# juliuspleunes4/TurboInfer

Hardware: AMD Instinct MI355X
Metric: decode tokens/s/GPU, Llama-7B-shape INT4 @2048 ctx; % HBM-read roofline (higher is better)
Workload: dtype w4a16; 1 GPU; llama2-7b INT4 g128 decode, 1 stream(s)/GPU, KV 2048, replay at pos 2047; model=llama2-7b, global_batch=1, seq_len=2048, parallelism=replicas1 (request-sharded, no collectives)

## Files before the change

include/ti_hip.h:

```cpp
#ifndef TI_HIP_H
#define TI_HIP_H

#include <stddef.h>
#include <stdint.h>

#ifdef __cplusplus
extern "C" {
#endif

typedef void* ti_stream_t;

enum ti_status {
  TI_OK = 0,
  TI_ERR_ARG = 1,
  TI_ERR_HIP = 2,
  TI_ERR_UNSUPPORTED = 3,
  TI_ERR_NOMEM = 4,
  TI_ERR_NODEV = 5
};

const char* ti_last_error(void);

int ti_device_count(int* count);
int ti_init(int device);
// ... 125 lines not shown
                      int max_seq, const int32_t* pos, int M, int heads, int kv_heads, int head_dim, int splits,
                      float* workspace, uint16_t* out, ti_stream_t s);
int ti_attn_decode_packed_f8(const float* q, const uint8_t* k_cache, const uint8_t* v_cache,
                             int64_t kv_stream_stride, int max_seq, const int32_t* pos, int M, int heads,
                             int kv_heads, int head_dim, int splits, float* workspace, uint16_t* out,
                             ti_stream_t s);
int ti_attn_decode_partials_f8(const float* q, const uint8_t* k_cache, const uint8_t* v_cache,
                               int64_t kv_stream_stride, int max_seq, const int32_t* pos, int M, int heads,
                               int kv_heads, int head_dim, int splits, uint16_t* part_o, float* part_ml,
                               ti_stream_t s);
int ti_qkv_attn_partials(const void* tiles, const uint16_t* scales, int bits, const uint16_t* fx,
                         const float* ss_in, int n_ss, float eps, const float* rope_cs, const int32_t* pos,
                         uint16_t* k_cache, uint16_t* v_cache, int max_seq, int K, int heads, int kv_heads,
                         int head_dim, int splits, uint16_t* part_o, float* part_ml, void* xchg, ti_stream_t s);
size_t ti_qkv_attn_part_o_elems(int heads, int head_dim, int splits);
size_t ti_qkv_attn_part_ml_elems(int heads, int head_dim, int splits);
size_t ti_qkv_attn_xchg_bytes(int heads, int splits);
size_t ti_qkv_attn_error_offset(int heads, int splits);
int ti_qkv_attn_supported(int bits, int K, int heads, int kv_heads, int head_dim, int splits);
int ti_attn_prefill(const float* q, const uint16_t* k_cache, const uint16_t* v_cache, int max_seq,
                    const int32_t* pos, int M, int heads, int kv_heads, int head_dim, uint16_t* out,
                    ti_stream_t s);
int ti_attn_prefill_f8(const float* q, const uint8_t* k_cache, const uint8_t* v_cache, int max_seq,
                       const int32_t* pos, int M, int heads, int kv_heads, int head_dim, uint16_t* out,
                       ti_stream_t s);
size_t ti_attn_prefill_split_workspace_bytes(int M, int heads, int head_dim, int splits);
int ti_attn_prefill_split(const float* q, const uint16_t* k_cache, const uint16_t* v_cache, int max_seq,
                          const int32_t* pos, int M, int heads, int kv_heads, int head_dim, int splits,
                          float* workspace, uint16_t* out, ti_stream_t s);
int ti_attn_prefill_set_kernel(int mode);

int ti_gemm_kernel_name(int bits, int x_kind, int M, int N, int K, char* buf, int len);

int ti_hbm_calibrate(size_t bytes, int reps, double* read_gbps, double* copy_gbps, ti_stream_t s);


typedef struct ti_step_args {
  const uint16_t* emb;
  float* h;
  int32_t hidden, M, vocab, in_stride, out_stride, placeholder_first;
  const int32_t* in_tokens;
  const int32_t* n_in;
  unsigned long long* argmax;
  int32_t* out_tokens;
  int32_t* pos;
  const int32_t* base_pos;
  const int32_t* step_ctr;
  const float* fold_w;
  uint16_t* fold_x;
  float* fold_ss;
} ti_step_args;
int ti_step_begin(const ti_step_args* a, ti_stream_t s);

#define TI_LA_STATE_WORDS 8
#define TI_LA_MAX_K 15
#define TI_LA_MAX_NGRAM 8
typedef struct ti_lookahead_args {
  int32_t* state;
  const int32_t* cfg;
  int32_t* hist;
  int32_t k, hidden, vocab, max_pos;
  const uint16_t* emb;
  float* h;
  int32_t* row_tok;
  int32_t* pos;
  unsigned long long* argmax;
// ... 41 lines not shown
```

turboinfer_amd/__init__.py:

```python
from __future__ import annotations

import ctypes as C
import os
import subprocess

import numpy as np

HERE = os.path.dirname(os.path.abspath(__file__))
ROOT = os.path.dirname(HERE)
LIB_PATH = os.environ.get("TI_LIB") or os.path.join(HERE, "lib", "libturboinfer_amd.so")

TI_OK = 0
X_F16, X_F32, X_F32_RMSNORM, X_F16_FOLDED, X_ATTN_SPLITS, X_F16_PACKED = 0, 1, 2, 3, 4, 5
ATTN_MAX_PART_SPLITS = 8
EPI_STORE_F32, EPI_STORE_F16, EPI_RESID_F32, EPI_SILU_MUL_F16, EPI_QKV_ROPE_KV, EPI_LOGITS_ARGMAX = range(6)
ARGMAX_SLOTS = 32
GEMM_MAX_ROWS = 1024
BITS_G32 = 32
BITS_AFF = 64
BITS_KV8 = 128
SCALE_GROUP, SCALE_TENSOR, SCALE_UNIT = 0, 1, 2
ROWS_CONCAT, ROWS_INTERLEAVE8 = 0, 1
(W_Q, W_K, W_V, W_O, W_GATE, W_UP, W_DOWN, W_LM_HEAD, V_ATTN_NORM, V_FFN_NORM, V_OUT_NORM, E_EMBED) = range(12)

# ... 39 lines not shown
                ("rope_theta", C.c_float), ("eps", C.c_float), ("bits", C.c_int32), ("max_seq", C.c_int32),
                ("max_batch", C.c_int32), ("compat", C.c_int32), ("device", C.c_int32),
                ("attn_splits", C.c_int32)]


EXPORTED = [
    "ti_last_error", "ti_device_count", "ti_init", "ti_device_name", "ti_malloc", "ti_free", "ti_memcpy_h2d",
    "ti_memcpy_d2h", "ti_memcpy_d2d", "ti_memset", "ti_stream_create", "ti_stream_destroy", "ti_stream_sync",
    "ti_device_sync", "ti_event_create", "ti_event_destroy", "ti_event_record", "ti_event_elapsed_ms",
    "ti_wpack_tile_bytes", "ti_wpack_scale_bytes", "ti_wpack_host", "ti_wsynth_device", "ti_fill_uniform_f16",
    "ti_fill_uniform_f32", "ti_fill_kv_uniform", "ti_kv_copy_slots", "ti_gemm_wq_a16", "ti_gemm_lds_bytes", "ti_gemm_prepare",
    "ti_gemm_max_rows", "ti_gemm_packed_rows", "ti_gemm_packed_rows_for", "ti_gemm_tile_plan", "ti_rmsnorm_f16", "ti_rmsnorm_f16_packed", "ti_attn_decode_packed", "ti_attn_prefill", "ti_attn_prefill_set_kernel",
    "ti_attn_workspace_bytes", "ti_attn_decode", "ti_step_begin", "ti_matmul_f32", "ti_rms_norm_f32",
    "ti_rope_f32", "ti_silu_f32", "ti_relu_f32", "ti_add_f32", "ti_mul_f32", "ti_softmax_f32", "ti_attention_f32",
    "ti_argmax_f32", "ti_engine_create", "ti_engine_destroy", "ti_engine_get_stream", "ti_engine_memory", "ti_engine_set_tensor",
    "ti_engine_synth", "ti_engine_fill_kv", "ti_engine_generate", "ti_engine_step", "ti_engine_compat_step",
    "ti_engine_replay_prepare", "ti_engine_set_prefill", "ti_engine_replay_run", "ti_engine_sync", "ti_engine_last_tokens",
    "ti_engine_time_kernel", "ti_engine_stamp_steps", "ti_rope_table", "ti_sample_token", 
    "ti_gemm_grid", "ti_engine_set_fold",
    "ti_attn_decode_partials", "ti_sample_device", "ti_sample_step", "ti_engine_generate_sampled",
    "ti_engine_beam_search", "ti_engine_serve", 
    "ti_wpack_q_host", "ti_engine_set_tensor_q", "ti_sample_workspace_bytes", "ti_sample_device_ws",
    "ti_wpack_q1_host", "ti_engine_set_tensor_q1", "ti_epilogue_bytes",
    "ti_sample_step_ws", "ti_hbm_calibrate", "ti_gemm_kernel_name",
    "ti_gemm_fold_partials", "ti_engine_set_stop", "ti_engine_counters",
    "ti_qkv_attn_partials", "ti_qkv_attn_part_o_elems", "ti_qkv_attn_part_ml_elems", "ti_engine_set_qkv_attn",
    "ti_qkv_attn_xchg_bytes", "ti_qkv_attn_supported", "ti_qkv_attn_error_offset",
    "ti_logprob_rows", "ti_engine_score",
    "ti_attn_decode_f8", "ti_attn_decode_packed_f8", "ti_attn_decode_partials_f8", "ti_fill_kv_uniform_f8",
    "ti_attn_prefill_f8", "ti_engine_prefill_attn_name",
    "ti_engine_read_kv",
    "ti_attn_prefill_split", "ti_attn_prefill_split_workspace_bytes", "ti_lookahead_begin", "ti_lookahead_accept",
    "ti_engine_generate_lookahead",
]

_lib = None


def build(jobs: int = 8) -> None:
    subprocess.run(["make", "-s", "-C", ROOT, f"-j{jobs}", "all"], check=True)


def lib() -> C.CDLL:
    global _lib
    if _lib is None:
        if not os.path.exists(LIB_PATH):
            raise TiError(f"native library missing: {LIB_PATH} (run `make` or __graft_entry__.build())")
        L = C.CDLL(LIB_PATH)
        vp, i32, i64, u64, f32, sz = C.c_void_p, C.c_int, C.c_int64, C.c_uint64, C.c_float, C.c_size_t
        L.ti_last_error.restype = C.c_char_p
        L.ti_device_count.argtypes = [C.POINTER(C.c_int)]
        L.ti_init.argtypes = [i32]
        L.ti_device_name.argtypes = [i32, C.c_char_p, i32]
        L.ti_malloc.argtypes = [C.POINTER(vp), sz]
        L.ti_free.argtypes = [vp]
        for n in ("ti_memcpy_h2d", "ti_memcpy_d2h", "ti_memcpy_d2d"):
            getattr(L, n).argtypes = [vp, vp, sz, vp]
        L.ti_memset.argtypes = [vp, i32, sz, vp]
        L.ti_stream_sync.argtypes = [vp]
        L.ti_wpack_tile_bytes.argtypes = [i32, i32, i32]
        L.ti_wpack_tile_bytes.restype = sz
        L.ti_wpack_scale_bytes.argtypes = [i32, i32, i32]
        L.ti_wpack_scale_bytes.restype = sz
        L.ti_wpack_host.argtypes = [vp, i32, i32, i32, i32, i32, i32, i32, vp, vp]
        L.ti_wsynth_device.argtypes = [u64, C.c_uint32, i32, i32, i32, i32, i32, i32, vp, vp, vp]
        L.ti_fill_uniform_f16.argtypes = [u64, C.c_uint32, u64, f32, vp, vp]
# ... 64 lines not shown
            L.ti_engine_set_fold.argtypes = [vp, i32, C.POINTER(C.c_int)]
        if hasattr(L, "ti_qkv_attn_partials"):
            L.ti_engine_set_qkv_attn.argtypes = [vp, i32, C.POINTER(C.c_int)]
            L.ti_qkv_attn_partials.argtypes = [vp, vp, i32, vp, vp, i32, f32, vp, vp, vp, vp, i32, i32, i32, i32,
                                               i32, i32, vp, vp, vp, vp]
            L.ti_qkv_attn_xchg_bytes.argtypes = [i32, i32]
            L.ti_qkv_attn_supported.argtypes = [i32, i32, i32, i32, i32, i32]
            L.ti_qkv_attn_xchg_bytes.restype = sz
            L.ti_qkv_attn_error_offset.argtypes = [i32, i32]
            L.ti_qkv_attn_error_offset.restype = sz
            L.ti_qkv_attn_part_o_elems.argtypes = [i32, i32, i32]
            L.ti_qkv_attn_part_o_elems.restype = sz
            L.ti_qkv_attn_part_ml_elems.argtypes = [i32, i32, i32]
            L.ti_qkv_attn_part_ml_elems.restype = sz
        if hasattr(L, "ti_engine_score"):
            L.ti_logprob_rows.argtypes = [vp, i32, i32, i32, vp, vp, vp, vp]
            L.ti_engine_score.argtypes = [vp, i32, vp, i32, i32, vp, vp, vp]
        if hasattr(L, "ti_attn_decode_f8"):
            for n in ("ti_attn_decode_f8", "ti_attn_decode_packed_f8", "ti_attn_decode_partials_f8"):
                getattr(L, n).argtypes = [vp, vp, vp, i64, i32, vp, i32, i32, i32, i32, i32, vp, vp, vp]
            L.ti_fill_kv_uniform_f8.argtypes = [u64, C.c_uint32, i32, i32, i32, i32, vp, vp]
            L.ti_engine_read_kv.argtypes = [vp, i32, i32, i32, i32, i32, vp]
        if hasattr(L, "ti_attn_prefill_f8"):
            L.ti_attn_prefill_f8.argtypes = [vp, vp, vp, i32, vp, i32, i32, i32, i32, vp, vp]
            L.ti_engine_prefill_attn_name.argtypes = [vp, i32, C.c_char_p, i32]
        if hasattr(L, "ti_engine_generate_lookahead"):
            L.ti_attn_prefill_split.argtypes = [vp, vp, vp, i32, vp, i32, i32, i32, i32, i32, vp, vp, vp]
            L.ti_attn_prefill_split_workspace_bytes.argtypes = [i32, i32, i32, i32]
            L.ti_attn_prefill_split_workspace_bytes.restype = sz
            L.ti_lookahead_begin.argtypes = [C.POINTER(LookaheadArgs), vp]
            L.ti_lookahead_accept.argtypes = [C.POINTER(LookaheadArgs), vp]
            L.ti_engine_generate_lookahead.argtypes = [vp, i32, vp, i32, i32, vp, i32, i32, i32, i32, vp,
                                                       C.POINTER(LookaheadStats)]
        L.ti_engine_compat_step.argtypes = [vp, i32, vp]
        L.ti_engine_replay_prepare.argtypes = [vp, i32, i32, i32]
        L.ti_engine_replay_run.argtypes = [vp, i32]
        L.ti_engine_sync.argtypes = [vp]
        L.ti_engine_last_tokens.argtypes = [vp, i32, vp]
        L.ti_engine_time_kernel.argtypes = [vp, i32, i32, i32, i32, C.POINTER(C.c_double), C.POINTER(C.c_double)]
        if hasattr(L, "ti_engine_stamp_steps"):
            L.ti_engine_stamp_steps.argtypes = [vp, i32, i32, vp, vp, C.POINTER(C.c_int)]
        L.ti_hbm_calibrate.argtypes = [sz, i32, C.POINTER(C.c_double), C.POINTER(C.c_double), vp]
        L.ti_gemm_kernel_name.argtypes = [i32, i32, i32, i32, i32, C.c_char_p, i32]
        L.ti_rope_table.argtypes = [vp, i32, i32, f32, vp]
        L.ti_sample_token.argtypes = [vp, i32, f32, i32, f32, f32, C.POINTER(C.c_int), C.POINTER(C.c_float)]
        _lib = L
    return _lib


def check(rc: int) -> None:
    if rc != TI_OK:
        raise TiError(f"ti error {rc}: {lib().ti_last_error().decode()}")


def device_count() -> int:
    n = C.c_int(0)
    check(lib().ti_device_count(C.byref(n)))
    return n.value


def init(device: int = 0) -> None:
    check(lib().ti_init(device))


def _ptr(a: np.ndarray) -> C.c_void_p:
    return C.c_void_p(a.ctypes.data)
# ... 311 lines not shown
```

turboinfer_amd/csrc/kernels/gemv.hip:

```cpp
#include <math.h>
#include <atomic>
#include <stdlib.h>

#include "common.hpp"
#include "attention_body.hpp"
#include "dequant.hpp"

namespace ti {

typedef uint32_t u32x4 __attribute__((ext_vector_type(4)));

#ifndef TI_GEMV_RING_VGPRS
#define TI_GEMV_RING_VGPRS 20
#endif
#ifndef TI_GEMV_SYNC
#define TI_GEMV_SYNC 0
#endif
#ifndef TI_GEMV_RING_DELAY
#define TI_GEMV_RING_DELAY 0
#endif
#ifndef TI_GEMV_EXP
#define TI_GEMV_EXP 0
#endif
#if TI_GEMV_EXP & 4
__device__ unsigned long long g_gemv_ts[4096 * 8];
#define GEMV_TS(k) \
  do { if (threadIdx.x == 0) g_gemv_ts[blockIdx.x * 8 + (k)] = __builtin_amdgcn_s_memrealtime(); } while (0)
__device__ unsigned long long g_gemv_wts[4096 * 8];
#define GEMV_WTS() \
  do { if ((threadIdx.x & 63) == 0) g_gemv_wts[blockIdx.x * 8 + (threadIdx.x >> 6)] = __builtin_amdgcn_s_memrealtime(); } while (0)
__device__ unsigned long long g_rows_ts[4096 * 8 * 8];
#define ROWS_TS(k)                                                                                     \
  do {                                                                                                 \
    if ((threadIdx.x & 63) == 0)                                                                       \
      g_rows_ts[(blockIdx.x * 8 + (threadIdx.x >> 6)) * 8 + (k)] = __builtin_amdgcn_s_memrealtime();   \
  } while (0)
#else
#define GEMV_WTS() do { } while (0)
#define GEMV_TS(k) do { } while (0)
#define ROWS_TS(k) do { } while (0)
#endif

constexpr int kGemvWaves = 8;
constexpr int kGemvThreads = kGemvWaves * kWave;

struct GemvArgs {
  const u32x4* tiles;
  const uint16_t* scales;
  const void* x;
  const float* norm_w;
  float eps;
  int32_t x_kind, ldx, M, N, K;
  ti_epilogue epi;
  unsigned long long* stamp;
};

__host__ __device__ constexpr int align16(int b) { return (b + 15) & ~15; }

struct GemmKnobs {
  bool splitk = true;
  bool rows_split = true;
};
__host__ inline const GemmKnobs& gemm_knobs() {
  static const GemmKnobs k = [] {
    GemmKnobs v;
    if (const char* e = getenv("TI_GEMM_SPLITK")) v.splitk = atoi(e) != 0;
    if (const char* e = getenv("TI_GEMM_ROWS_SPLIT")) v.rows_split = atoi(e) != 0;
    return v;
  }();
  return k;
}


__host__ __device__ inline int gemv_lds_bytes_tiles(int M, int K, int tiles_per_wg, bool g32 = false, bool aff = false);

__host__ inline int gemv_grid(int M, int N, int K, int num_cus, bool g32 = false, bool aff = false) {
  const int NT = N >> 4;
  const int g = num_cus > 0 ? num_cus : 256;
  int grid = NT < g ? NT : g;
  while (grid < NT && gemv_lds_bytes_tiles(M, K, (NT + grid - 1) / grid, g32, aff) > 160 * 1024) grid += grid / 8 + 1;
  return grid < NT ? grid : NT;
}

struct GemvLds {
  int x, sc, corr, slab, es, best, total, mins, bsum;
};
__host__ __device__ inline GemvLds gemv_lds_layout(int M, int K, int ntl, bool g32 = false, bool aff = false) {
  GemvLds l;
  const int gm = g32 ? 4 : 1;
  l.x = 0;
  l.sc = l.x + align16(M * (K + 8) * 2);
  l.mins = l.sc + align16(ntl * (K >> 7) * 32 * gm);
  l.corr = l.mins + (aff ? align16(ntl * (K >> 7) * 32 * gm) : 0);
  l.bsum = l.corr + (K >> 7) * 16 * 4 * gm;
  l.slab = l.bsum + (aff ? (K >> 7) * 16 * 4 * gm : 0);
  l.es = l.slab + (ntl + 1) * kGemvWaves * kWave * 16;
  const int es_bytes = 2 * ntl * M * 16 * 4 > M * 128 * 4 + 64 ? 2 * ntl * M * 16 * 4 : M * 128 * 4 + 64;
  l.best = l.es + align16(es_bytes);
  l.total = l.best + 16 * 8;
  return l;
// ... 124 lines not shown
      }
      break;
    }
    default:
      break;
  }
}

#ifndef TI_GEMV_NT
#define TI_GEMV_NT 1
#endif
__device__ __forceinline__ u32x4 ld_w(const u32x4* p) {
#if TI_GEMV_NT || (TI_GEMV_EXP & 16)
  return __builtin_nontemporal_load(p);
#else
  return *p;
#endif
}

__device__ __forceinline__ float int4_x_prep(f16x8& h) {
  const f16 s16 = (f16)0.0625f;
  h[2] *= s16; h[3] *= s16; h[6] *= s16; h[7] *= s16;
  const float lo = ((float)h[0] + (float)h[1]) + ((float)h[4] + (float)h[5]);
  const float hi = ((float)h[2] + (float)h[3]) + ((float)h[6] + (float)h[7]);
  return 1032.0f * lo + 1152.0f * hi;
}

__device__ __forceinline__ void lds_barrier() {
  asm volatile("s_waitcnt lgkmcnt(0)" ::: "memory");
  __builtin_amdgcn_s_barrier();
  asm volatile("" ::: "memory");
}

template <int BITS, int XM, bool G32 = false, bool AFF = false>
__global__ __launch_bounds__(kGemvThreads, 1) void gemv_wq_kernel(const u32x4* p_tiles, const uint16_t* p_scales,
                                                                   const void* p_x, const float* p_aux, int p_mgk,
                                                                   int p_N, int p_kx, int p_ldo, const float* p_pre,
                                                                   GemvArgs a) {
  const unsigned long long t_entry = stamp_now();
  const unsigned bid = blockIdx.x;
  a.tiles = p_tiles;
  a.scales = p_scales;
  a.x = p_x;
  a.norm_w = p_aux;
  a.M = p_mgk & 63;
  const int nt_q = p_N & 0xff, nt_r = (int)((unsigned)p_N >> 8);
  a.K = p_kx & 0xffff;
  a.ldx = XM == XM_F16F || XM == XM_ATTN ? a.K : (int)((unsigned)p_kx >> 16);
  const int p_grid = (p_mgk >> 6) & 0xfff;
  a.N = 16 * (nt_q * p_grid + nt_r);
  constexpr int C = TileFmt<BITS>::kChunks;
  constexpr int R = TI_GEMV_RING_VGPRS / (4 * C) > 2 ? TI_GEMV_RING_VGPRS / (4 * C) : 2;
  constexpr int XPF = 3;
  extern __shared__ __attribute__((aligned(16))) char smem[];
  GEMV_TS(0);
  const int KT = a.K >> 7, xs = a.K + 8, NT = a.N >> 4, K8 = a.K >> 3;
  const int tid = threadIdx.x, lane = tid & 63;
  const int wave = __builtin_amdgcn_readfirstlane(tid >> 6);
  const int t0 = (int)bid * nt_q + ((int)bid < nt_r ? (int)bid : nt_r);
  const int ntl = nt_q + ((int)bid < nt_r ? 1 : 0);
  constexpr bool kOneRow = XM == XM_F16F || XM == XM_ATTN || XM == XM_NORM1;
  const int KW = wave < KT ? (KT - wave + kGemvWaves - 1) / kGemvWaves : 0;
  const int total = ntl * KW;
  static_assert(!G32 || BITS != 16, "group-32 weights: int4 / int8");
  static_assert(!AFF || (G32 && BITS == 4), "affine blocks: group-32 int4");
  const GemvLds L = gemv_lds_layout(a.M, a.K, ntl, G32, AFF);
  uint16_t* ml = (uint16_t*)(smem + L.mins);
// ... 27 lines not shown
  u32x4 po[XM == XM_ATTN ? kPS : 1];
  float2 pml[XM == XM_ATTN ? kPS : 1];
  auto load_x = [&]() {
    if constexpr (XM == XM_ATTN) {
      const int S = (int)((unsigned)p_kx >> 16), hsh = ((p_mgk >> 21) & 3) == 2 ? 7 : 6;
      const int i = tid < K8 ? tid : K8 - 1, h = (8 * i) >> hsh, d = (8 * i) & ((1 << hsh) - 1);
#pragma unroll
      for (int sp = 0; sp < kPS; ++sp) {
        const int r = h * S + (sp < S ? sp : S - 1);
        po[sp] = *(const u32x4*)((const f16*)a.x + ((size_t)r << hsh) + d);
        pml[sp] = *(const float2*)(p_aux + 2 * r);
      }
    } else if constexpr (XM == XM_NORM1) {
      const int k8 = tid < K8 ? tid : K8 - 1;
      const float* xr = (const float*)a.x;
      v0 = *(const float4*)(xr + 8 * k8);
      v1 = *(const float4*)(xr + 8 * k8 + 4);
    } else if constexpr (XM == XM_F16 || XM == XM_F16F) {
#pragma unroll
      for (int q = 0; q < XPF; ++q) {
        const int i = tid + q * kGemvThreads < nx16 ? tid + q * kGemvThreads : nx16 - 1;
        const int m = kOneRow ? 0 : i / K8, k8 = i - m * K8;
        xr16[q] = *(const u32x4*)((const f16*)a.x + (size_t)m * a.ldx + 8 * k8);
      }
    }
  };
  if constexpr (XM == XM_NORM1) {
#endif
    const int k8 = tid < K8 ? tid : K8 - 1;
    w0 = *(const float4*)(a.norm_w + 8 * k8);
    w1 = *(const float4*)(a.norm_w + 8 * k8 + 4);
  }
  load_x();
  const int kind = (p_mgk >> 18) & 7, ldo = p_ldo;
  const int n_res = kind == TI_EPI_RESID_F32 ? ntl * a.M * 16 : 0;
  const float* pre_p;
  {
    const int idx = tid < n_res ? tid : 0;
    const int tl = kOneRow ? idx >> 4 : idx / (a.M * 16), rem = idx - tl * a.M * 16, m = rem >> 4, n = rem & 15;
    pre_p = kind == TI_EPI_RESID_F32 ? p_pre + (size_t)m * ldo + (t0 + tl) * 16 + n
            : kind == TI_EPI_QKV_ROPE_KV ? p_pre + (tid < a.M ? tid : 0) : p_pre;
  }
  const float pre = *pre_p;
  float fw_pre = 0.0f;
  float ss4[4] = {0.0f, 0.0f, 0.0f, 0.0f};
  const int n_ss = (int)((unsigned)p_kx >> 16);
  if constexpr (XM == XM_F16F) {
#pragma unroll
    for (int j = 0; j < 4; ++j) ss4[j] = p_aux[lane + 64 * j < n_ss ? lane + 64 * j : 0];
  }

  const u32x4* tb = a.tiles + (size_t)t0 * KT * (kWave * C) + lane;
  const size_t last_off = total > 0 ? ((size_t)(ntl - 1) * KT + wave + kGemvWaves * (KW - 1)) * (kWave * C) : 0;
  int rt = 0, rk = 0, rj = 0;
  auto refill_off = [&]() -> size_t {
    const size_t o = rj < total ? ((size_t)rt * KT + wave + kGemvWaves * rk) * (kWave * C) : last_off;
    ++rj;
    if (++rk == KW) { rk = 0; ++rt; }
    return o;
  };
  constexpr int R0 = R >= 8 ? 4 : R;
  u32x4 ring[R][C];
#if TI_GEMV_RING_DELAY > 0
  __builtin_amdgcn_s_sleep(TI_GEMV_RING_DELAY);
#endif
#pragma unroll
  for (int s = 0; s < R0; ++s) {
    const size_t o = refill_off();
#pragma unroll
    for (int c = 0; c < C; ++c) ring[s][c] = ld_w(tb + o + c * kWave);
  }
  const bool fold = (XM == XM_F16 || XM == XM_ATTN) && kind == TI_EPI_RESID_F32 && a.epi.fold_x != nullptr;
// ... 65 lines not shown
  } else if constexpr (XM == XM_F16 || XM == XM_F16F) {
#pragma unroll
    for (int q = 0; q < XPF; ++q) {
      const int i = tid + q * kGemvThreads;
      const int m = kOneRow || i >= nx16 ? 0 : i / K8, k8 = i - m * K8;
      float part = 0.0f;
      if (i < nx16) {
        if (kRegPrep && reg_prep) {
          f16x8 h = __builtin_bit_cast(f16x8, xr16[q]);
          part = int4_x_prep(h);
          *(f16x8*)(xl + m * xs + 8 * k8) = h;
        } else {
          *(u32x4*)(xl + m * xs + 8 * k8) = xr16[q];
        }
      }
      if (kRegPrep && reg_prep) {
        part = group_sum<16>(part);
        if (i < nx16 && (lane & 15) == 0) corr[(k8 >> 4) * 16 + m] = part;
      }
    }
  }
  if constexpr (BITS != 16) {
    for (int i = tid + kGemvThreads; i < n_sc; i += kGemvThreads) ((u32x4*)sl)[i] = sg[i];
  }
  if constexpr (AFF) {
    const u32x4* mg = (const u32x4*)(a.scales + (size_t)NT * KT * 64 + (size_t)t0 * KT * 64);
    for (int i = tid; i < n_sc; i += kGemvThreads) ((u32x4*)ml)[i] = mg[i];
  }
  if constexpr (XM == XM_F16 || XM == XM_F16F) {
    if (nx16 > XPF * kGemvThreads) stage_x_generic<XM>(a, xl, red, XPF * kGemvThreads);
  } else if constexpr (XM != XM_NORM1 && XM != XM_ATTN) {
    stage_x_generic<XM>(a, xl, red, 0);
  }
  if (a.epi.kind == TI_EPI_QKV_ROPE_KV && tid < a.M) ((int*)(es + a.M * a.epi.head_dim))[tid] = __builtin_bit_cast(int, pre);
  if (tid < 16) best_l[tid] = 0ull;
  lds_barrier();
  STAMP_MARK(ph_staged);
#pragma unroll
  for (int s = R0; s < R; ++s) {
    const size_t o = refill_off();
#pragma unroll
    for (int c = 0; c < C; ++c) ring[s][c] = ld_w(tb + o + c * kWave);
  }
  if constexpr (BITS == 4) if (!reg_prep) {
    const f16 s16 = (f16)0.0625f;
    for (int i0 = 0; i0 < a.M * K8; i0 += kGemvThreads) {
      const int idx = i0 + tid;
      float part = 0.0f, sx = 0.0f;
      int m = 0, k8 = 0;
      if (idx < a.M * K8) {
        m = idx / K8;
        k8 = idx - m * K8;
        f16x8 h = *(const f16x8*)(xl + m * xs + 8 * k8);
        h[2] *= s16; h[3] *= s16; h[6] *= s16; h[7] *= s16;
        *(f16x8*)(xl + m * xs + 8 * k8) = h;
        const float lo = ((float)h[0] + (float)h[1]) + ((float)h[4] + (float)h[5]);
        const float hi = ((float)h[2] + (float)h[3]) + ((float)h[6] + (float)h[7]);
        part = 1032.0f * lo + 1152.0f * hi;
        if constexpr (AFF) sx = lo + 16.0f * hi;
      }
      if constexpr (G32) {
        part = group_sum<4>(part);
        if (idx < a.M * K8 && (lane & 3) == 0) corr[(k8 >> 2) * 16 + m] = part;
        if constexpr (AFF) {
          sx = group_sum<4>(sx);
          if (idx < a.M * K8 && (lane & 3) == 0) bsum[(k8 >> 2) * 16 + m] = sx;
        }
      } else {
        part = group_sum<16>(part);
        if (idx < a.M * K8 && (lane & 15) == 0) corr[(k8 >> 4) * 16 + m] = part;
      }
    }
    lds_barrier();
  }

  float cs_reg = 0.0f;
  const int n_cs = a.epi.kind == TI_EPI_QKV_ROPE_KV ? a.M * a.epi.head_dim : 0;
  if (n_cs > 0) {
    const int hd = a.epi.head_dim, idx = tid < n_cs ? tid : 0, m = idx / hd, j = idx - m * hd;
    cs_reg = a.epi.rope_cs[(size_t)((const int*)(es + a.M * hd))[m] * hd + j];
  }

  GEMV_TS(2);
  STAMP_MARK(ph_stream);
  const int r = lane & 15, kq = lane >> 4;
  const f16* xrow = xl + (r < a.M ? r : a.M - 1) * xs + kq * 32;
  f32x4 acc = {0.0f, 0.0f, 0.0f, 0.0f};
  uint32_t magic;
  asm volatile("v_mov_b32 %0, 0x64006400" : "=v"(magic));
  f32x4* my_slab = slab + wave * kWave + lane;
  constexpr int kSlabStride = kGemvWaves * kWave;
  int ct = 0, ck = 0;
  auto item = [&](const u32x4 (&w)[C]) {
    const int kt = wave + kGemvWaves * ck;
    f32x4 t = {0.0f, 0.0f, 0.0f, 0.0f};
    if constexpr (BITS == 16) t = acc;
    if constexpr (G32) {
      const f16* xr32 = xrow - kq * 32 + kq * 8;
#pragma unroll
      for (int s4 = 0; s4 < 4; ++s4) {
        const f16x8 bf = dequant_step<BITS>(w, s4, magic);
        const f16x8 af = *(const f16x8*)(xr32 + kt * 128 + s4 * 32);
        f32x4 tb = __builtin_amdgcn_mfma_f32_16x16x32_f16(af, bf, (f32x4){0.0f, 0.0f, 0.0f, 0.0f}, 0, 0, 0);
        if constexpr (BITS == 4) tb -= *(const f32x4*)(corr + (kt * 4 + s4) * 16 + 4 * kq);
        const float sc = h2f(sl[((ct * KT + kt) * 4 + s4) * 16 + r]);
        acc[0] = fmaf(sc, tb[0], acc[0]);
        acc[1] = fmaf(sc, tb[1], acc[1]);
        acc[2] = fmaf(sc, tb[2], acc[2]);
        acc[3] = fmaf(sc, tb[3], acc[3]);
        if constexpr (AFF) {
          const float mt = fmaf(8.0f, sc, h2f(ml[((ct * KT + kt) * 4 + s4) * 16 + r]));
          const f32x4 bs = *(const f32x4*)(bsum + (kt * 4 + s4) * 16 + 4 * kq);
          acc[0] = fmaf(mt, bs[0], acc[0]);
// ... 40 lines not shown
  int blk = 0;
  for (; j0 + R <= common; j0 += R) {
#pragma unroll
    for (int s = 0; s < R; ++s) {
      item(ring[s]);
      const size_t o = refill_off();
#pragma unroll
      for (int c = 0; c < C; ++c) ring[s][c] = ld_w(tb + o + c * kWave);
    }
    if (++blk == TI_GEMV_SYNC) {
      blk = 0;
      __builtin_amdgcn_s_barrier();
    }
  }
#endif
  for (; j0 + R <= total; j0 += R) {
#pragma unroll
    for (int s = 0; s < R; ++s) {
      item(ring[s]);
      const size_t o = refill_off();
#pragma unroll
      for (int c = 0; c < C; ++c) ring[s][c] = ld_w(tb + o + c * kWave);
    }
  }
#pragma unroll
  for (int s = 0; s < R; ++s)
    if (j0 + s < total) item(ring[s]);
  if (KW == 0)
    for (int tl = 0; tl < ntl; ++tl) my_slab[tl * kSlabStride] = (f32x4){0.0f, 0.0f, 0.0f, 0.0f};

  GEMV_TS(3);
  GEMV_WTS();
  STAMP_MARK(ph_streamed);
  if (tid < n_res) es[tid] = pre;
  if (fold && tid < n_res) es[n_res + tid] = fw_pre;
  if (tid < n_cs) es[tid] = cs_reg;
  for (int i = tid + kGemvThreads; i < n_res; i += kGemvThreads) {
    const int tl = i / (a.M * 16), rem = i - tl * a.M * 16, m = rem >> 4, n = rem & 15;
    es[i] = p_pre[(size_t)m * ldo + (t0 + tl) * 16 + n];
    if (fold) es[n_res + i] = a.epi.fold_w[(size_t)t0 * 16 + i];
  }
  float rms = 1.0f;
  if constexpr (XM == XM_F16F) {
    float t = 0.0f;
#pragma unroll
    for (int j = 0; j < 4; ++j) t += lane + 64 * j < n_ss ? ss4[j] : 0.0f;
    t = group_sum<kWave>(t);
    rms = sqrtf(t / (float)a.K + a.eps);
  }
  float ssacc = 0.0f;
  const float* fw_l = es + n_res;
  for (int i = tid + kGemvThreads; i < n_cs; i += kGemvThreads) {
    const int hd = a.epi.head_dim, m = i / hd, j = i - m * hd;
    es[i] = a.epi.rope_cs[(size_t)((const int*)(es + a.M * hd))[m] * hd + j];
  }
  lds_barrier();
  GEMV_TS(5);
  STAMP_MARK(ph_reduce);
  unsigned long long best[4] = {0ull, 0ull, 0ull, 0ull};
  if (a.M <= 4) {
    for (int tb0 = wave * kWave; tb0 < ntl * 16; tb0 += kGemvThreads) {
      const int t = tb0 + lane, ok = t < ntl * 16, tl = ok ? t >> 4 : 0, n = lane & 15;
      const f32x4* sp = slab + tl * kSlabStride + n;
      f32x4 v = sp[0];
#pragma unroll
      for (int w = 1; w < kGemvWaves; ++w) v += sp[w * kWave];
// ... 1213 lines not shown
}

__host__ inline bool splitk_on() { return gemm_knobs().splitk; }
__host__ inline size_t splitk_slab_bytes(int n_ks, int n_cb, int n_rb, int tpw) {
  return (size_t)n_ks * n_cb * n_rb * kGemvWaves * tpw * 4 * kWave * 16;
}
__host__ inline void tile_plan(int M, int N, int K, bool g32, int cus, int64_t ws_bytes, int* wmr_o, int* tpw_o,
                               int* ks_o, int* rb_o = nullptr) {
  const int shape = tile_shape(M, N, K, g32, cus);
  const int wmr = (shape >> 3) & 3, tpw = shape & 7, rb = shape & 32 ? 2 : 4;
  *wmr_o = wmr;
  *tpw_o = tpw;
  *ks_o = 1;
  if (rb_o) *rb_o = rb;
  if (rb == 2 || !splitk_on() || ws_bytes <= TI_SPLITK_TICKET_BYTES) return;
  const int NT = N >> 4, KT = K >> 7, cols = (8 / wmr) * tpw;
  const int n_cb = (NT + cols - 1) / cols, n_rb = (M + 64 * wmr - 1) / (64 * wmr);
  const long wgs = (long)n_cb * n_rb, grid1 = (long)(n_cb + 7) / 8 * 8 * n_rb;
  if (wgs * 4 > cus || (size_t)wgs * kGemvWaves * 4 > TI_SPLITK_TICKET_BYTES) return;
  int S = (int)(cus / grid1);
  while (S > 1 && ((KT + S - 1) / S < 8 || splitk_slab_bytes(S, n_cb, n_rb, tpw) + TI_SPLITK_TICKET_BYTES > (size_t)ws_bytes))
    --S;
  *ks_o = S;
}

__host__ inline int gemv_xmode(int x_kind, int M, int K) {
  if (x_kind == TI_X_F16) return XM_F16;
  if (x_kind == TI_X_F16_FOLDED) return XM_F16F;
  if (x_kind == TI_X_ATTN_SPLITS) return XM_ATTN;
  if (x_kind == TI_X_F32) return XM_F32;
  return M == 1 && (K >> 3) <= kGemvThreads ? XM_NORM1 : XM_NORM;
}

template <int BITS, bool G32 = false, bool AFF = false>
static int launch_gemv(const GemvArgs& a, int lds, hipStream_t s, int grid) {
  const float* pre = a.epi.kind == TI_EPI_RESID_F32 ? (const float*)a.epi.out
                     : a.epi.kind == TI_EPI_QKV_ROPE_KV ? (const float*)a.epi.pos : (const float*)a.x;
  const int xm = gemv_xmode(a.x_kind, a.M, a.K);
  const float* aux = xm == XM_F16F || xm == XM_ATTN ? a.epi.ss_in : xm == XM_F16 ? nullptr : a.norm_w;
  const int mgk = a.M | (grid << 6) | (a.epi.kind << 18) | (xm == XM_ATTN ? (a.epi.head_dim / 64) << 21 : 0);
  const int kx = a.K | ((xm == XM_F16F || xm == XM_ATTN ? a.epi.n_ss : a.ldx) << 16);
  const int ldo = a.epi.ldo;
  const int NT = a.N >> 4, nt_q = NT / grid, nt_r = NT % grid;
  if (nt_q > 255 || nt_r >= (1 << 23))
    return ti_set_error(TI_ERR_UNSUPPORTED, "gemv_wq_kernel: %d tiles over %d workgroups", NT, grid);
  const int pn = nt_q | (nt_r << 8);
  switch (xm) {
    case XM_F16: hipLaunchKernelGGL((gemv_wq_kernel<BITS, XM_F16, G32, AFF>), dim3(grid), dim3(kGemvThreads), lds, s, a.tiles, a.scales, a.x, aux, mgk, pn, kx, ldo, pre, a); break;
    case XM_F32: hipLaunchKernelGGL((gemv_wq_kernel<BITS, XM_F32, G32, AFF>), dim3(grid), dim3(kGemvThreads), lds, s, a.tiles, a.scales, a.x, aux, mgk, pn, kx, ldo, pre, a); break;
    case XM_ATTN: hipLaunchKernelGGL((gemv_wq_kernel<BITS, XM_ATTN, G32, AFF>), dim3(grid), dim3(kGemvThreads), lds, s, a.tiles, a.scales, a.x, aux, mgk, pn, kx, ldo, pre, a); break;
    case XM_F16F: hipLaunchKernelGGL((gemv_wq_kernel<BITS, XM_F16F, G32, AFF>), dim3(grid), dim3(kGemvThreads), lds, s, a.tiles, a.scales, a.x, aux, mgk, pn, kx, ldo, pre, a); break;
    case XM_NORM1: hipLaunchKernelGGL((gemv_wq_kernel<BITS, XM_NORM1, G32, AFF>), dim3(grid), dim3(kGemvThreads), lds, s, a.tiles, a.scales, a.x, aux, mgk, pn, kx, ldo, pre, a); break;
    default: hipLaunchKernelGGL((gemv_wq_kernel<BITS, XM_NORM, G32, AFF>), dim3(grid), dim3(kGemvThreads), lds, s, a.tiles, a.scales, a.x, aux, mgk, pn, kx, ldo, pre, a); break;
  }
  TI_LAUNCH_CHECK("gemv_wq_kernel");
  return TI_OK;
}

__global__ __launch_bounds__(kGemvThreads) void rmsnorm_f16_kernel(const float* x, int ldx, const float* w, float eps,
                                                                    uint16_t* y, int ldy, int K, int pk_kt) {
  __shared__ float red[kGemvWaves];
  const int m = blockIdx.x, tid = threadIdx.x, K8 = K >> 3;
  const float* xr = x + (size_t)m * ldx;
  float ss = 0.0f;
  for (int k8 = tid; k8 < K8; k8 += kGemvThreads) {
    const float4 v0 = *(const float4*)(xr + 8 * k8), v1 = *(const float4*)(xr + 8 * k8 + 4);
    ss = fmaf(v0.x, v0.x, ss); ss = fmaf(v0.y, v0.y, ss); ss = fmaf(v0.z, v0.z, ss); ss = fmaf(v0.w, v0.w, ss);
    ss = fmaf(v1.x, v1.x, ss); ss = fmaf(v1.y, v1.y, ss); ss = fmaf(v1.z, v1.z, ss); ss = fmaf(v1.w, v1.w, ss);
  }
  ss = group_sum<kWave>(ss);
  if ((tid & 63) == 0) red[tid >> 6] = ss;
  __syncthreads();
  float tot = 0.0f;
#pragma unroll
  for (int i = 0; i < kGemvWaves; ++i) tot += red[i];
  const float rms = sqrtf(tot / (float)K + eps);
  for (int k8 = tid; k8 < K8; k8 += kGemvThreads) {
    const float4 v0 = *(const float4*)(xr + 8 * k8), v1 = *(const float4*)(xr + 8 * k8 + 4);
    const float4 w0 = *(const float4*)(w + 8 * k8), w1 = *(const float4*)(w + 8 * k8 + 4);
// ... 146 lines not shown

static std::atomic<unsigned long long> g_prepared{0};

}

static int query_cus() {
  int n = ti::g_num_cus.load(std::memory_order_relaxed);
  if (n <= 0) {
    int dev = 0;
    if (!(hipGetDevice(&dev) == hipSuccess &&
          hipDeviceGetAttribute(&n, hipDeviceAttributeMultiprocessorCount, dev) == hipSuccess && n > 0))
      n = 256;
    ti::g_num_cus.store(n, std::memory_order_relaxed);
  }
  return n;
}

extern "C" int ti_gemm_prepare(void) {
  using namespace ti;
  query_cus();
  int dev = 0;
  TI_HIP_CHECK(hipGetDevice(&dev), "hipGetDevice");
  const unsigned long long bit = 1ull << (dev & 63);
  if (g_prepared.load(std::memory_order_acquire) & bit) return TI_OK;
  const void* fns[] = {
      (const void*)gemv_wq_kernel<4, XM_F16>,  (const void*)gemv_wq_kernel<4, XM_F32>,
      (const void*)gemv_wq_kernel<4, XM_NORM1>, (const void*)gemv_wq_kernel<4, XM_NORM>,
      (const void*)gemv_wq_kernel<8, XM_F16>,  (const void*)gemv_wq_kernel<8, XM_F32>,
      (const void*)gemv_wq_kernel<8, XM_NORM1>, (const void*)gemv_wq_kernel<8, XM_NORM>,
      (const void*)gemv_wq_kernel<16, XM_F16>, (const void*)gemv_wq_kernel<16, XM_F32>,
      (const void*)gemv_wq_kernel<16, XM_NORM1>, (const void*)gemv_wq_kernel<16, XM_NORM>,
      (const void*)gemv_wq_kernel<4, XM_F16F>, (const void*)gemv_wq_kernel<8, XM_F16F>,
      (const void*)gemv_wq_kernel<16, XM_F16F>, (const void*)gemv_wq_kernel<4, XM_ATTN>,
      (const void*)gemv_wq_kernel<8, XM_ATTN>, (const void*)gemv_wq_kernel<16, XM_ATTN>, TI_MB_FNS, TI_ROWS_FNS,
      TI_TILE_FNS};
  for (const void* f : fns)
    TI_HIP_CHECK(hipFuncSetAttribute(f, hipFuncAttributeMaxDynamicSharedMemorySize, 160 * 1024),
                 "hipFuncSetAttribute(gemv_wq_kernel)");
  g_prepared.fetch_or(bit, std::memory_order_acq_rel);
  return TI_OK;
}

extern "C" int ti_gemm_lds_bytes(int M, int N, int K) {
  if (M < 1 || N < 16 || K < 128) return 0;
  const int NT = N >> 4, grid = ti::gemv_grid(M, N, K, query_cus());
  return ti::gemv_lds_bytes_tiles(M, K, (NT + grid - 1) / grid);
}

static int fused_rows_pref(int bits) { return bits == 4 ? 2 : 16; }
static bool fused_fits(int M, int N, int K, bool g32 = false, bool aff = false) {
  if (M > 16) return false;
  const int NT = N >> 4, grid = ti::gemv_grid(M, N, K, query_cus(), g32, aff);
  return ti::gemv_lds_bytes_tiles(M, K, (NT + grid - 1) / grid, g32, aff) <= 160 * 1024;
}
static bool use_batched(int bits, int x_kind, int M, int N, int K) {
  const bool mb_ok = bits == 4 && x_kind == TI_X_F16;
  return !fused_fits(M, N, K) || (mb_ok && M > fused_rows_pref(bits));
}

static bool wide_tile(int bits, int M, int N) {
  constexpr long kWideMN = 850000, kWideN32 = 16384;
  if (bits != 4 || M <= 16 || M >= ti::tile_rows()) return false;
  if (M <= 32 && ti::tile_rb2_on() && N >= kWideN32) return true;
  return (long)M * N >= kWideMN;
}
extern "C" int ti_gemm_packed_rows(int bits, int M) { return bits == 4 && M > 16 && M < ti::tile_rows() ? 1 : 0; }
extern "C" int ti_gemm_packed_rows_for(int bits, int M, int N, int K) {
  (void)K;
// ... 219 lines not shown
  if (tile) {
    const void* f = tile_fn(tpw, g32, wmr, xbuf, trb);
    void* args[] = {&a, &n_cb, &n_rb, &n_ks};
    TI_HIP_CHECK(hipLaunchKernel(f, dim3(grid), dim3(kGemvThreads), args, lds, s), "hipLaunchKernel(gemm_tile_kernel)");
    TI_LAUNCH_CHECK("gemm_tile_kernel");
    return TI_OK;
  }
  if (rows) return launch_rows(a, rMB, rRG, ntl, grid, r_rb, lds, s, g32);
  if (batched) return launch_mb(a, M > 16 ? 2 : 1, grid, ntl, lds, s);
  if (aff) return launch_gemv<4, true, true>(a, lds, s, grid);
  if (g32) return bits == 4 ? launch_gemv<4, true>(a, lds, s, grid) : launch_gemv<8, true>(a, lds, s, grid);
  if (bits == 4) return launch_gemv<4>(a, lds, s, grid);
  if (bits == 8) return launch_gemv<8>(a, lds, s, grid);
  return launch_gemv<16>(a, lds, s, grid);
}

extern "C" int ti_epilogue_bytes(void) { return (int)sizeof(ti_epilogue); }

extern "C" int ti_gemm_kernel_name(int bits, int x_kind, int M, int N, int K, char* buf, int len) {
  using namespace ti;
  if (!buf || len < 1) return ti_set_error(TI_ERR_ARG, "ti_gemm_kernel_name: null buffer");
  if ((bits != 4 && bits != 8 && bits != 16) || M < 1 || M > TI_GEMM_MAX_ROWS || N < 16 || K < 128)
    return ti_set_error(TI_ERR_ARG, "ti_gemm_kernel_name: bits %d M %d N %d K %d", bits, M, N, K);
  const bool packed_x = x_kind == TI_X_F16_PACKED;
  const bool batched = packed_x || use_batched(bits, x_kind, M, N, K);
  const bool tile = batched && x_kind == TI_X_F16 && (M >= tile_rows() || wide_tile(bits, M, N));
  const bool rows = !tile && batched && (packed_x || M > 32 || (M > 16 && rows_on()));
  const char* name = tile ? "gemm_tile_kernel" : rows ? "gemm_rows_kernel" : batched ? (mb_use_lds(M > 16 ? 2 : 1) ? "gemv_mb_kernel" : "gemv_mbr_kernel") : nullptr;
  if (name) snprintf(buf, (size_t)len, "%s", name);
  else snprintf(buf, (size_t)len, "gemv_wq_kernel<%d,%d>", bits, gemv_xmode(x_kind, M, K));
  return TI_OK;
}

extern "C" int ti_gemm_grid(int M, int N, int K) {
  if (M < 1 || M > 16 || N < 16 || K < 128 || (N & 15) || (K & 127) || !fused_fits(M, N, K)) return 0;
  return ti::gemv_grid(M, N, K, query_cus());
}

extern "C" int ti_gemm_wq_a16(const void* tiles, const uint16_t* scales, int bits, const void* x,
                              int x_kind, int ldx, const float* norm_w, float eps, int M, int N, int K,
                              const ti_epilogue* epi, ti_stream_t stream) {
  return gemm_impl(tiles, scales, bits, x, x_kind, ldx, norm_w, eps, M, N, K, epi, stream);
}
```

Measured before the change: 811.4 tokens/s.

## Specialize one-row GEMV kernels per epilogue kind with register-direct epilogues

Adds an EPI template parameter to the GEMV kernel so batch-1 decode launches compile a variant specialized for each epilogue (residual, SiLU-mul, QKV RoPE/KV write, logits argmax). The specialized path reduces the per-wave partials and applies the epilogue directly from registers, precomputing output pointers and RoPE coefficients before the weight stream. This skips the generic LDS staging and epilogue dispatch after streaming. It adds more kernel instantiations, a launch counter, and an env knob to fall back to the generic path.

```diff
diff --git a/include/ti_hip.h b/include/ti_hip.h
--- a/include/ti_hip.h
+++ b/include/ti_hip.h
@@ -181,6 +181,8 @@
 
 int ti_gemm_kernel_name(int bits, int x_kind, int M, int N, int K, char* buf, int len);
 
+uint64_t ti_gemm_onerow_epi_launches(void);
+
 int ti_hbm_calibrate(size_t bytes, int reps, double* read_gbps, double* copy_gbps, ti_stream_t s);
 
 
diff --git a/turboinfer_amd/__init__.py b/turboinfer_amd/__init__.py
--- a/turboinfer_amd/__init__.py
+++ b/turboinfer_amd/__init__.py
@@ -95,6 +95,7 @@
     "ti_engine_read_kv",
     "ti_attn_prefill_split", "ti_attn_prefill_split_workspace_bytes", "ti_lookahead_begin", "ti_lookahead_accept",
     "ti_engine_generate_lookahead",
+    "ti_gemm_onerow_epi_launches",
 ]
 
 _lib = None
@@ -225,6 +226,9 @@
             L.ti_lookahead_accept.argtypes = [C.POINTER(LookaheadArgs), vp]
             L.ti_engine_generate_lookahead.argtypes = [vp, i32, vp, i32, i32, vp, i32, i32, i32, i32, vp,
                                                        C.POINTER(LookaheadStats)]
+        if hasattr(L, "ti_gemm_onerow_epi_launches"):
+            L.ti_gemm_onerow_epi_launches.argtypes = []
+            L.ti_gemm_onerow_epi_launches.restype = u64
         L.ti_engine_compat_step.argtypes = [vp, i32, vp]
         L.ti_engine_replay_prepare.argtypes = [vp, i32, i32, i32]
         L.ti_engine_replay_run.argtypes = [vp, i32]
diff --git a/turboinfer_amd/csrc/kernels/gemv.hip b/turboinfer_amd/csrc/kernels/gemv.hip
--- a/turboinfer_amd/csrc/kernels/gemv.hip
+++ b/turboinfer_amd/csrc/kernels/gemv.hip
@@ -18,6 +18,9 @@
 #endif
 #ifndef TI_GEMV_RING_DELAY
 #define TI_GEMV_RING_DELAY 0
+#endif
+#ifndef TI_GEMV_ONEROW_RMS_EARLY
+#define TI_GEMV_ONEROW_RMS_EARLY 0
 #endif
 #ifndef TI_GEMV_EXP
 #define TI_GEMV_EXP 0
@@ -60,12 +63,14 @@
 struct GemmKnobs {
   bool splitk = true;
   bool rows_split = true;
+  bool epi_generic = false;
 };
 __host__ inline const GemmKnobs& gemm_knobs() {
   static const GemmKnobs k = [] {
     GemmKnobs v;
     if (const char* e = getenv("TI_GEMM_SPLITK")) v.splitk = atoi(e) != 0;
     if (const char* e = getenv("TI_GEMM_ROWS_SPLIT")) v.rows_split = atoi(e) != 0;
+    if (const char* e = getenv("TI_GEMV_EPI_GENERIC")) v.epi_generic = atoi(e) != 0;
     return v;
   }();
   return k;
@@ -256,7 +261,7 @@
   asm volatile("" ::: "memory");
 }
 
-template <int BITS, int XM, bool G32 = false, bool AFF = false>
+template <int BITS, int XM, bool G32 = false, bool AFF = false, int EPI = -1>
 __global__ __launch_bounds__(kGemvThreads, 1) void gemv_wq_kernel(const u32x4* p_tiles, const uint16_t* p_scales,
                                                                    const void* p_x, const float* p_aux, int p_mgk,
                                                                    int p_N, int p_kx, int p_ldo, const float* p_pre,
@@ -350,12 +355,12 @@
     w1 = *(const float4*)(a.norm_w + 8 * k8 + 4);
   }
   load_x();
-  const int kind = (p_mgk >> 18) & 7, ldo = p_ldo;
+  const int kind = EPI >= 0 ? EPI : (p_mgk >> 18) & 7, ldo = p_ldo;
   const int n_res = kind == TI_EPI_RESID_F32 ? ntl * a.M * 16 : 0;
   const float* pre_p;
   {
     const int idx = tid < n_res ? tid : 0;
-    const int tl = kOneRow ? idx >> 4 : idx / (a.M * 16), rem = idx - tl * a.M * 16, m = rem >> 4, n = rem & 15;
+    const int tl = kOneRow || EPI >= 0 ? idx >> 4 : idx / (a.M * 16), rem = idx - tl * a.M * 16, m = rem >> 4, n = rem & 15;
     pre_p = kind == TI_EPI_RESID_F32 ? p_pre + (size_t)m * ldo + (t0 + tl) * 16 + n
             : kind == TI_EPI_QKV_ROPE_KV ? p_pre + (tid < a.M ? tid : 0) : p_pre;
   }
@@ -487,7 +492,7 @@
   } else if constexpr (XM != XM_NORM1 && XM != XM_ATTN) {
     stage_x_generic<XM>(a, xl, red, 0);
   }
-  if (a.epi.kind == TI_EPI_QKV_ROPE_KV && tid < a.M) ((int*)(es + a.M * a.epi.head_dim))[tid] = __builtin_bit_cast(int, pre);
+  if ((EPI >= 0 ? kind : a.epi.kind) == TI_EPI_QKV_ROPE_KV && tid < a.M) ((int*)(es + a.M * a.epi.head_dim))[tid] = __builtin_bit_cast(int, pre);
   if (tid < 16) best_l[tid] = 0ull;
   lds_barrier();
   STAMP_MARK(ph_staged);
@@ -530,10 +535,52 @@
   }
 
   float cs_reg = 0.0f;
-  const int n_cs = a.epi.kind == TI_EPI_QKV_ROPE_KV ? a.M * a.epi.head_dim : 0;
+  const int n_cs = EPI < 0 && a.epi.kind == TI_EPI_QKV_ROPE_KV ? a.M * a.epi.head_dim : 0;
   if (n_cs > 0) {
     const int hd = a.epi.head_dim, idx = tid < n_cs ? tid : 0, m = idx / hd, j = idx - m * hd;
     cs_reg = a.epi.rope_cs[(size_t)((const int*)(es + a.M * hd))[m] * hd + j];
+  }
+
+  const bool o_ok = tid < ntl * 16;
+  const int o_tl = o_ok ? tid >> 4 : 0, o_ng = (t0 + o_tl) * 16 + (lane & 15);
+  [[maybe_unused]] float o_rms = 1.0f;
+  [[maybe_unused]] void* o_out = nullptr;
+  [[maybe_unused]] uint16_t* o_fx = nullptr;
+  [[maybe_unused]] float2 o_cs = {1.0f, 0.0f};
+  [[maybe_unused]] int o_rot = 0;
+  [[maybe_unused]] uint32_t o_ci = 0;
+  if constexpr (EPI >= 0) {
+    if constexpr (XM == XM_F16F && TI_GEMV_ONEROW_RMS_EARLY) {
+      float t = 0.0f;
+#pragma unroll
+      for (int j = 0; j < 4; ++j) t += lane + 64 * j < n_ss ? ss4[j] : 0.0f;
+      t = group_sum<kWave>(t);
+      o_rms = sqrtf(t / (float)a.K + a.eps);
+    }
+    if constexpr (EPI == TI_EPI_RESID_F32) {
+      o_out = (void*)pre_p;
+      if (fold) o_fx = a.epi.fold_x + o_ng;
+    } else if constexpr (EPI == TI_EPI_SILU_MUL_F16) {
+      o_out = (uint16_t*)a.epi.out + (t0 + o_tl) * 8 + (lane & 7);
+    } else if constexpr (EPI == TI_EPI_LOGITS_ARGMAX) {
+      o_out = (float*)a.epi.out + o_ng;
+    } else if constexpr (EPI == TI_EPI_QKV_ROPE_KV) {
+      const ti_epilogue& e = a.epi;
+      const int hd = e.head_dim, p = ((const int*)(es + hd))[0];
+      const bool is_q = o_ng < e.q_dim, qk = o_ng < e.q_dim + e.kv_dim;
+      const int c = o_ng - (is_q ? 0 : e.q_dim) - (qk ? 0 : e.kv_dim);
+      const int kvh = c / hd, d = c - kvh * hd;
+      if (qk) {
+        o_rot = 1 + (d & 1);
+        o_cs = *(const float2*)(e.rope_cs + (size_t)p * hd + (d & ~1));
+      }
+      if (is_q) {
+        o_out = (float*)e.out + o_ng;
+      } else {
+        o_out = qk ? e.k_cache : e.v_cache;
+        o_ci = (uint32_t)((kvh * e.max_seq + p) * hd + d);
+      }
+    }
   }
 
   GEMV_TS(2);
@@ -640,6 +687,90 @@
   GEMV_TS(3);
   GEMV_WTS();
   STAMP_MARK(ph_streamed);
+  if constexpr (EPI >= 0) {
+    if constexpr (XM == XM_F16F && !TI_GEMV_ONEROW_RMS_EARLY) {
+      float t = 0.0f;
+#pragma unroll
+      for (int j = 0; j < 4; ++j) t += lane + 64 * j < n_ss ? ss4[j] : 0.0f;
+      t = group_sum<kWave>(t);
+      o_rms = sqrtf(t / (float)a.K + a.eps);
+    }
+    lds_barrier();
+    STAMP_MARK(ph_reduce);
+    float ssacc = 0.0f;
+    if (wave * kWave < ntl * 16) {
+      const float* sp = (const float*)(slab + o_tl * kSlabStride + (lane & 15));
+      float pw[kGemvWaves];
+#pragma unroll
+      for (int w = 0; w < kGemvWaves; ++w) pw[w] = sp[w * kWave * 4];
+      float v = pw[0];
+#pragma unroll
+      for (int w = 1; w < kGemvWaves; ++w) v += pw[w];
+      if constexpr (XM == XM_F16F) v = v / o_rms;
+      if constexpr (EPI == TI_EPI_RESID_F32) {
+        if (o_ok) {
+          const float r = pre + v;
+          *(float*)o_out = r;
+          if (fold) {
+            *o_fx = f2h(r * fw_pre);
+            ssacc = fmaf(r, r, ssacc);
+          }
+        }
+      } else if constexpr (EPI == TI_EPI_SILU_MUL_F16) {
+        const float up = lane_xor<8>(v);
+        const float s = v / (1.0f + expf(-v));
+        if (o_ok && (lane & 8) == 0) *(uint16_t*)o_out = f2h(up * s);
+      } else if constexpr (EPI == TI_EPI_QKV_ROPE_KV) {
+        const float partner = lane_xor<1>(v);
+        float r = v;
+        if (o_rot == 1) r = fmaf(-partner, o_cs.y, v * o_cs.x);
+        else if (o_rot == 2) r = fmaf(v, o_cs.x, partner * o_cs.y);
+        if (o_ok) {
+          if (o_ng < a.epi.q_dim) *(float*)o_out = r;
+          else if (a.epi.kv_fp8) ((uint8_t*)o_out)[o_ci] = f2e4m3(r);
+          else ((uint16_t*)o_out)[o_ci] = f2h(r);
+        }
+      } else if constexpr (EPI == TI_EPI_LOGITS_ARGMAX) {
+        unsigned long long best = 0ull;
+        if (o_ok) {
+          *(float*)o_out = v;
+          best = ((unsigned long long)float_order_key(v) << 32) | (unsigned long long)(0xFFFFFFFFu - (uint32_t)o_ng);
+        }
+#pragma unroll
+        for (int o = 1; o < kWave; o <<= 1) {
+          const unsigned long long other = __shfl_xor(best, o, kWave);
+          best = other > best ? other : best;
+        }
+        if (lane == 0 && best) atomicMax(a.epi.argmax + (bid & (TI_ARGMAX_SLOTS - 1)), best);
+      }
+    }
+    STAMP_MARK(ph_epi);
+    if constexpr (EPI == TI_EPI_LOGITS_ARGMAX) {
+      if (a.epi.step_ctr && bid == 0 && tid == 0) *a.epi.step_ctr += a.epi.advance;
+    }
+    if constexpr (EPI == TI_EPI_RESID_F32) {
+      if (fold && ntl * 16 <= kWave) {
+        if (wave == 0) {
+          const float sw = group_sum<kWave>(ssacc);
+          if (lane == 0) a.epi.fold_ss[bid] = sw;
+        }
+      } else if (fold) {
+        float* red2 = (float*)best_l;
+        const float sw = group_sum<kWave>(ssacc);
+        if (lane == 0) red2[wave] = sw;
+        lds_barrier();
+        if (tid == 0) {
+          float t = 0.0f;
+#pragma unroll
+          for (int w = 0; w < kGemvWaves; ++w) t += red2[w];
+          a.epi.fold_ss[bid] = t;
+        }
+      }
+    }
+    GEMV_TS(4);
+    stamp_end(a.stamp, t_entry, ph_issued, ph_staged, ph_stream, ph_streamed, ph_reduce, ph_epi, ph_streamed);
+    return;
+  }
   if (tid < n_res) es[tid] = pre;
   if (fold && tid < n_res) es[n_res + tid] = fw_pre;
   if (tid < n_cs) es[tid] = cs_reg;
@@ -1919,6 +2050,16 @@
   return M == 1 && (K >> 3) <= kGemvThreads ? XM_NORM1 : XM_NORM;
 }
 
+static std::atomic<unsigned long long> g_onerow_epi_launches{0};
+__host__ inline bool onerow_epi(const GemvArgs& a, int xm, int grid) {
+  if (gemm_knobs().epi_generic || a.M != 1) return false;
+  if (xm != XM_F16F && xm != XM_ATTN && xm != XM_F16 && xm != XM_NORM1) return false;
+  const int NT = a.N >> 4;
+  if ((NT + grid - 1) / grid * 16 > kGemvThreads) return false;
+  if (a.epi.kind == TI_EPI_QKV_ROPE_KV && (long long)a.epi.kv_dim * a.epi.max_seq > 0x7fffffffll) return false;
+  return true;
+}
+
 template <int BITS, bool G32 = false, bool AFF = false>
 static int launch_gemv(const GemvArgs& a, int lds, hipStream_t s, int grid) {
   const float* pre = a.epi.kind == TI_EPI_RESID_F32 ? (const float*)a.epi.out
@@ -1932,6 +2073,27 @@
   if (nt_q > 255 || nt_r >= (1 << 23))
     return ti_set_error(TI_ERR_UNSUPPORTED, "gemv_wq_kernel: %d tiles over %d workgroups", NT, grid);
   const int pn = nt_q | (nt_r << 8);
+  if constexpr (BITS != 16 && !G32 && !AFF) {
+#define TI_ONEROW(XMODE, KIND)                                                                                  \
+  if (xm == XMODE && a.epi.kind == KIND) {                                                                      \
+    hipLaunchKernelGGL((gemv_wq_kernel<BITS, XMODE, false, false, KIND>), dim3(grid), dim3(kGemvThreads), lds, s, \
+                       a.tiles, a.scales, a.x, aux, mgk, pn, kx, ldo, pre, a);                                  \
+    TI_LAUNCH_CHECK("gemv_wq_kernel");                                                                          \
+    g_onerow_epi_launches.fetch_add(1, std::memory_order_relaxed);                                              \
+    return TI_OK;                                                                                               \
+  }
+    if (onerow_epi(a, xm, grid)) {
+      TI_ONEROW(XM_F16F, TI_EPI_SILU_MUL_F16)
+      TI_ONEROW(XM_F16F, TI_EPI_LOGITS_ARGMAX)
+      TI_ONEROW(XM_F16F, TI_EPI_QKV_ROPE_KV)
+      TI_ONEROW(XM_ATTN, TI_EPI_RESID_F32)
+      TI_ONEROW(XM_F16, TI_EPI_RESID_F32)
+      TI_ONEROW(XM_NORM1, TI_EPI_SILU_MUL_F16)
+      TI_ONEROW(XM_NORM1, TI_EPI_LOGITS_ARGMAX)
+      TI_ONEROW(XM_NORM1, TI_EPI_QKV_ROPE_KV)
+    }
+#undef TI_ONEROW
+  }
   switch (xm) {
     case XM_F16: hipLaunchKernelGGL((gemv_wq_kernel<BITS, XM_F16, G32, AFF>), dim3(grid), dim3(kGemvThreads), lds, s, a.tiles, a.scales, a.x, aux, mgk, pn, kx, ldo, pre, a); break;
     case XM_F32: hipLaunchKernelGGL((gemv_wq_kernel<BITS, XM_F32, G32, AFF>), dim3(grid), dim3(kGemvThreads), lds, s, a.tiles, a.scales, a.x, aux, mgk, pn, kx, ldo, pre, a); break;
@@ -2144,8 +2306,19 @@
       (const void*)gemv_wq_kernel<16, XM_NORM1>, (const void*)gemv_wq_kernel<16, XM_NORM>,
       (const void*)gemv_wq_kernel<4, XM_F16F>, (const void*)gemv_wq_kernel<8, XM_F16F>,
       (const void*)gemv_wq_kernel<16, XM_F16F>, (const void*)gemv_wq_kernel<4, XM_ATTN>,
-      (const void*)gemv_wq_kernel<8, XM_ATTN>, (const void*)gemv_wq_kernel<16, XM_ATTN>, TI_MB_FNS, TI_ROWS_FNS,
-      TI_TILE_FNS};
+      (const void*)gemv_wq_kernel<8, XM_ATTN>, (const void*)gemv_wq_kernel<16, XM_ATTN>,
+#define TI_ONEROW_FNS(B)                                                            \
+  (const void*)gemv_wq_kernel<B, XM_F16F, false, false, TI_EPI_SILU_MUL_F16>,       \
+  (const void*)gemv_wq_kernel<B, XM_F16F, false, false, TI_EPI_LOGITS_ARGMAX>,      \
+  (const void*)gemv_wq_kernel<B, XM_F16F, false, false, TI_EPI_QKV_ROPE_KV>,        \
+  (const void*)gemv_wq_kernel<B, XM_ATTN, false, false, TI_EPI_RESID_F32>,          \
+  (const void*)gemv_wq_kernel<B, XM_F16, false, false, TI_EPI_RESID_F32>,           \
+  (const void*)gemv_wq_kernel<B, XM_NORM1, false, false, TI_EPI_SILU_MUL_F16>,      \
+  (const void*)gemv_wq_kernel<B, XM_NORM1, false, false, TI_EPI_LOGITS_ARGMAX>,     \
+  (const void*)gemv_wq_kernel<B, XM_NORM1, false, false, TI_EPI_QKV_ROPE_KV>
+      TI_ONEROW_FNS(4), TI_ONEROW_FNS(8),
+#undef TI_ONEROW_FNS
+      TI_MB_FNS, TI_ROWS_FNS, TI_TILE_FNS};
   for (const void* f : fns)
     TI_HIP_CHECK(hipFuncSetAttribute(f, hipFuncAttributeMaxDynamicSharedMemorySize, 160 * 1024),
                  "hipFuncSetAttribute(gemv_wq_kernel)");
@@ -2431,6 +2604,10 @@
   return TI_OK;
 }
 
+extern "C" uint64_t ti_gemm_onerow_epi_launches(void) {
+  return ti::g_onerow_epi_launches.load(std::memory_order_relaxed);
+}
+
 extern "C" int ti_gemm_grid(int M, int N, int K) {
   if (M < 1 || M > 16 || N < 16 || K < 128 || (N & 15) || (K & 127) || !fused_fits(M, N, K)) return 0;
   return ti::gemv_grid(M, N, K, query_cus());
```

Result: faster. 844.4 tokens/s (median of 6 runs) (+4.1%).
